# jskvrna/MonoSOWA

Measured on AMD Instinct MI355X. Metric: MonoDETR training img/s (KITTI 1280x384), higher is better.
Workload: dtype f32; 1 GPU; MonoDETR resnet50 KITTI 1280x384, fwd+criterion+bwd+AdamW step, per-GPU batch 16, synthetic images + random pseudo-labels; global_batch=16, per_gpu_batch=16, parallelism=dp1, accumulation_micro_steps=1, mixed_cameras=False, queries=550, tuned=True

## Files before the change

### include/monosowa_pointwise.h

```cpp
#ifndef MONOSOWA_POINTWISE_H_
#define MONOSOWA_POINTWISE_H_
#ifdef __cplusplus
extern "C" {
#endif

int mono_set_deterministic(int on);

int mono_bias_act_f32(float *y, const float *bias, const float *residual, long long rows, int C, int relu, void *stream);
int mono_bias_relu_maxpool_nhwc_f32(const float *y, const float *bias, float *out, int N, int H, int W, int C, void *stream);
int mono_conv1x1_tail_f32(const float *x, const float *b_in, const float *w, const float *b_out, const float *res, float *y,
                          long long M, int K, int N, void *stream);
int mono_conv1x1_tail_ds_f32(const float *x, const float *b_in, const float *w, const float *x0, const float *wd, const float *b_out,
                             float *y, long long M, int K, int N, void *stream);
int mono_conv1x1_head_f32(const float *x, const float *w, const float *b_out, float *y, long long M, int K, int N, void *stream);

int mono_relu_grad_f32(const float *grad_out, const float *y, float *grad_in, long long n, void *stream);
int mono_relu_grad_scale_f32(const float *grad_out, const float *y, const float *scale, float *grad_in, long long n, int C, void *stream);

int mono_bias_relu_mask_f32(float *y, const float *bias, const float *residual, unsigned char *mask, long long rows, int C,
                            void *stream);
int mono_relu_grad_mask_f32(const float *grad_a, const float *grad_b, const unsigned char *mask, float *grad_in, long long n,
                            void *stream);
int mono_relu_grad_mask3_f32(const float *grad_a, const float *grad_b, const float *grad_c, const unsigned char *mask, float *grad_in,
                             long long n, void *stream);

int mono_affine_relu_mask_f32(float *y, const float *scale, const float *shift, unsigned char *mask, long long rows, int C,
                              void *stream);
int mono_affine_relu_grad_f32(const float *grad, const unsigned char *mask, const float *scale, float *grad_in, long long rows,
                              int C, void *stream);

int mono_relu_grad2_f32(const float *grad_a, const float *grad_b, const float *y, float *grad_in, long long n, void *stream);
int mono_relu_grad3_f32(const float *grad_a, const float *grad_b, const float *grad_c, const float *y, float *grad_in, long long n,
                        void *stream);

int mono_dropout_add_layernorm_fwd_f32(const float *x, const float *z, const float *gamma, const float *beta, float *y,
                                       float *s, float *mean, float *rstd, long long rows, int C, float p,
                                       unsigned long long seed, float eps, void *stream);

int mono_relu_dropout_fwd_f32(const float *h, float *y, long long n, float p, unsigned long long seed, void *stream);
int mono_relu_dropout_bwd_f32(const float *grad_y, const float *y, float *grad_h, long long n, float p, void *stream);
int mono_relu_dropout_bwd_colsum_f32(const float *grad_y, const float *y, float *grad_h, float *colsum, float *partials, long long rows,
                                     float p, void *stream);

int mono_matched_losses_fwd_f32(const float *boxes, const float *depth, const float *dims, const float *angle,
                                const long long *idx, const float *t_box, const float *t_depth, const float *t_size,
                                const long long *t_bin, const float *t_res, float *out, float *comp, int NL, int B, int Q,
                                int K, void *stream);
int mono_matched_losses_bwd_f32(const float *boxes, const float *depth, const float *dims, const float *angle,
                                const long long *idx, const float *t_box, const float *t_depth, const float *t_size,
                                const long long *t_bin, const float *t_res, const float *comp, const float *grad_out,
                                float *g_boxes, float *g_depth, float *g_dims, float *g_angle, int NL, int B, int Q, int K,
                                void *stream);

int mono_adamw_step_f32(const void *table, int n_chunks, double beta1, double beta2, double eps, double step_size, void *stream);

long long mono_linear_wgrad_workspace(int R, int M, int N);
int mono_linear_wgrad_f32(const float *dy, long long ldy, const float *x, long long ldx, float *dw, float *db, float *ws, int R, int M,
                          int N, void *stream);

int mono_colsum_any_blocks(long long rows);
int mono_colsum_any_f32(const float *g, float *out, float *partials, long long rows, int C, void *stream);

// ... 69 lines not shown
```

### monosowa_amd/csrc/pointwise.hip

```cpp
#include <hip/hip_runtime.h>

#include "groupnorm.hip"
#include "matched_losses.hip"
#include "ddn_loss.hip"
#include "head_tail.hip"
#include "lsap_device.hip"
#include "conv1x1_fused.hip"
#include "small_wgrad.hip"
#include <stdint.h>
#include <algorithm>

namespace mono {

template <bool RELU, bool RES>
__global__ __launch_bounds__(256) void bias_act_kernel(float *__restrict__ y, const float *__restrict__ bias,
                                                       const float *__restrict__ residual, long long n_vec, int c_vec) {
  const long long stride = (long long)gridDim.x * blockDim.x;
  for (long long i = (long long)blockIdx.x * blockDim.x + threadIdx.x; i < n_vec; i += stride) {
    float4 v = reinterpret_cast<float4 *>(y)[i];
    const float4 b = reinterpret_cast<const float4 *>(bias)[i % c_vec];
    v.x += b.x; v.y += b.y; v.z += b.z; v.w += b.w;
    if (RES) {
      const float4 r = reinterpret_cast<const float4 *>(residual)[i];
      v.x += r.x; v.y += r.y; v.z += r.z; v.w += r.w;
    }
    if (RELU) { v.x = fmaxf(v.x, 0.f); v.y = fmaxf(v.y, 0.f); v.z = fmaxf(v.z, 0.f); v.w = fmaxf(v.w, 0.f); }
    reinterpret_cast<float4 *>(y)[i] = v;
  }
}

__global__ __launch_bounds__(256) void bias_relu_maxpool_kernel(const float *__restrict__ y, const float *__restrict__ bias,
                                                                float *__restrict__ out, int N, int H, int W, int c_vec, int OH, int OW) {
  const long long n_items = (long long)N * OH * OW * c_vec, stride = (long long)gridDim.x * blockDim.x;
  for (long long i = (long long)blockIdx.x * blockDim.x + threadIdx.x; i < n_items; i += stride) {
    const int c = (int)(i % c_vec);
    long long t = i / c_vec;
    const int ox = (int)(t % OW);
    t /= OW;
    const int oy = (int)(t % OH), n = (int)(t / OH);
    float4 m = make_float4(-INFINITY, -INFINITY, -INFINITY, -INFINITY);
#pragma unroll
    for (int dy = 0; dy < 3; ++dy) {
      const int iy = 2 * oy - 1 + dy;
      if (iy < 0 || iy >= H) continue;
#pragma unroll
      for (int dx = 0; dx < 3; ++dx) {
        const int ix = 2 * ox - 1 + dx;
        if (ix < 0 || ix >= W) continue;
        const float4 v = reinterpret_cast<const float4 *>(y)[(((long long)n * H + iy) * W + ix) * c_vec + c];
        m.x = fmaxf(m.x, v.x); m.y = fmaxf(m.y, v.y); m.z = fmaxf(m.z, v.z); m.w = fmaxf(m.w, v.w);
      }
    }
    const float4 b = reinterpret_cast<const float4 *>(bias)[c];
    reinterpret_cast<float4 *>(out)[i] = make_float4(fmaxf(m.x + b.x, 0.f), fmaxf(m.y + b.y, 0.f), fmaxf(m.z + b.z, 0.f), fmaxf(m.w + b.w, 0.f));
  }
}

template <bool RES>
__global__ __launch_bounds__(256) void bias_relu_mask_kernel(float *__restrict__ y, const float *__restrict__ bias,
                                                             const float *__restrict__ residual, unsigned char *__restrict__ mask,
// ... 455 lines not shown
      adamw_one(P.y, G.y, M.y, V.y, wd, b1, omb1, b2, omb2, eps, neg);
      adamw_one(P.z, G.z, M.z, V.z, wd, b1, omb1, b2, omb2, eps, neg);
      adamw_one(P.w, G.w, M.w, V.w, wd, b1, omb1, b2, omb2, eps, neg);
      reinterpret_cast<float4 *>(p)[i] = P; reinterpret_cast<float4 *>(m)[i] = M; reinterpret_cast<float4 *>(v)[i] = V;
    }
    for (int i = (n4 << 2) + threadIdx.x; i < n; i += 256) adamw_one(p[i], g[i], m[i], v[i], wd, b1, omb1, b2, omb2, eps, neg);
  } else {
    for (int i = threadIdx.x; i < n; i += 256) adamw_one(p[i], g[i], m[i], v[i], wd, b1, omb1, b2, omb2, eps, neg);
  }
}

inline int grid_for_vec(long long n_vec) {
  long long g = (n_vec + 255) / 256;
  if (g > 256LL * 32) g = 256LL * 32;
  return (int)(g < 1 ? 1 : g);
}

}

static int g_deterministic = 0;

extern "C" {

int mono_set_deterministic(int on) {
  const int prev = g_deterministic;
  g_deterministic = on != 0;
  return prev;
}

int mono_reduce_blocks(long long rows);

int mono_bias_act_f32(float *y, const float *bias, const float *residual, long long rows, int C, int relu, void *stream_) {
  if (!y || !bias) return -1;
  if (rows <= 0 || C <= 0 || (C & 3) || ((uintptr_t)y & 15) || ((uintptr_t)bias & 15) || ((uintptr_t)residual & 15)) return -2;
  hipStream_t stream = (hipStream_t)stream_;
  const long long n_vec = rows * C / 4;
  const int g = mono::grid_for_vec(n_vec);
  if (relu && residual) mono::bias_act_kernel<true, true><<<g, 256, 0, stream>>>(y, bias, residual, n_vec, C / 4);
  else if (relu) mono::bias_act_kernel<true, false><<<g, 256, 0, stream>>>(y, bias, nullptr, n_vec, C / 4);
  else if (residual) mono::bias_act_kernel<false, true><<<g, 256, 0, stream>>>(y, bias, residual, n_vec, C / 4);
  else mono::bias_act_kernel<false, false><<<g, 256, 0, stream>>>(y, bias, nullptr, n_vec, C / 4);
  return (int)hipGetLastError();
}

int mono_bias_relu_maxpool_nhwc_f32(const float *y, const float *bias, float *out, int N, int H, int W, int C, void *stream_) {
  if (!y || !bias || !out) return -1;
  if (N <= 0 || H <= 0 || W <= 0 || C <= 0 || (C & 3) || ((uintptr_t)y & 15) || ((uintptr_t)bias & 15) || ((uintptr_t)out & 15)) return -2;
  const int OH = (H - 1) / 2 + 1, OW = (W - 1) / 2 + 1;
  const long long n_items = (long long)N * OH * OW * (C / 4);
  mono::bias_relu_maxpool_kernel<<<mono::grid_for_vec(n_items), 256, 0, (hipStream_t)stream_>>>(y, bias, out, N, H, W, C / 4, OH, OW);
  return (int)hipGetLastError();
}

int mono_conv1x1_tail_f32(const float *x, const float *b_in, const float *w, const float *b_out, const float *res, float *y,
                          long long M, int K, int N, void *stream_) {
  if (!x || !b_in || !w || !b_out || !res || !y) return -1;
  if (M <= 0 || K != mono::kC1K || N != mono::kC1N) return -2;
  if (((uintptr_t)x & 15) || ((uintptr_t)w & 15) || ((uintptr_t)res & 15) || ((uintptr_t)y & 15)) return -2;
  if ((const float *)y == res || (const float *)y == x) return -2;
  const long long strips = (M + 31) / 32, per_wg = mono::kC1Threads / 64;
  const int grid = (int)std::min<long long>(512, (strips + per_wg - 1) / per_wg);
  mono::conv1x1_tail_kernel<<<grid, mono::kC1Threads, 0, (hipStream_t)stream_>>>(x, b_in, w, b_out, res, y, M);
  return (int)hipGetLastError();
}

int mono_conv1x1_tail_ds_f32(const float *x, const float *b_in, const float *w, const float *x0, const float *wd, const float *b_out,
                             float *y, long long M, int K, int N, void *stream_) {
  if (!x || !b_in || !w || !x0 || !wd || !b_out || !y) return -1;
  if (M <= 0 || K != mono::kC1K || N != mono::kC1N) return -2;
  if (((uintptr_t)x & 15) || ((uintptr_t)w & 15) || ((uintptr_t)x0 & 15) || ((uintptr_t)wd & 15) || ((uintptr_t)y & 15)) return -2;
  if ((const float *)y == x || (const float *)y == x0) return -2;
  const long long strips = (M + 31) / 32, per_wg = mono::kC1Threads2 / 64;
  const int grid = (int)std::min<long long>(256, (strips + per_wg - 1) / per_wg);
  mono::conv1x1_tail_ds_kernel<<<grid, mono::kC1Threads2, 0, (hipStream_t)stream_>>>(x, b_in, w, x0, wd, b_out, y, M);
  return (int)hipGetLastError();
}

int mono_conv1x1_head_f32(const float *x, const float *w, const float *b_out, float *y, long long M, int K, int N, void *stream_) {
  if (!x || !w || !b_out || !y) return -1;
  if (M <= 0 || (K != 64 && K != 256) || N != 64) return -2;
  if (((uintptr_t)x & 15) || ((uintptr_t)w & 15) || ((uintptr_t)y & 15)) return -2;
  const long long strips = (M + 31) / 32, per_wg = mono::kC1Threads / 64;
  const int grid = (int)std::min<long long>(512, (strips + per_wg - 1) / per_wg);
  if (K == 64) mono::conv1x1_head_kernel<64><<<grid, mono::kC1Threads, 0, (hipStream_t)stream_>>>(x, w, b_out, y, M);
  else mono::conv1x1_head_kernel<256><<<grid, mono::kC1Threads, 0, (hipStream_t)stream_>>>(x, w, b_out, y, M);
  return (int)hipGetLastError();
}

int mono_bias_relu_mask_f32(float *y, const float *bias, const float *residual, unsigned char *mask, long long rows, int C,
                            void *stream_) {
  if (!y || !bias || !mask) return -1;
  if (rows <= 0 || C <= 0 || (C & 3) || ((uintptr_t)y & 15) || ((uintptr_t)bias & 15) || ((uintptr_t)residual & 15)) return -2;
  const long long n_vec = rows * C / 4;
  const int g = mono::grid_for_vec(n_vec);
  if (residual) mono::bias_relu_mask_kernel<true><<<g, 256, 0, (hipStream_t)stream_>>>(y, bias, residual, mask, n_vec, C / 4);
  else mono::bias_relu_mask_kernel<false><<<g, 256, 0, (hipStream_t)stream_>>>(y, bias, nullptr, mask, n_vec, C / 4);
  return (int)hipGetLastError();
}

int mono_affine_relu_mask_f32(float *y, const float *scale, const float *shift, unsigned char *mask, long long rows, int C,
                              void *stream_) {
  if (!y || !scale || !shift || !mask) return -1;
  if (rows <= 0 || C <= 0 || (C & 3) || ((uintptr_t)y & 15) || ((uintptr_t)scale & 15) || ((uintptr_t)shift & 15)) return -2;
  const long long n_vec = rows * C / 4;
  mono::affine_relu_mask_kernel<<<mono::grid_for_vec(n_vec), 256, 0, (hipStream_t)stream_>>>(y, scale, shift, mask, n_vec, C / 4);
  return (int)hipGetLastError();
// ... 453 lines not shown
```

### monosowa_amd/monodetr/backbone.py

```python
import os

import torch
import torch.nn.functional as F
from torch import nn

from ..pointwise import (affine_relu, affine_relu_supported, bias_act, bias_act_fork, bias_relu_maxpool,
                         bias_relu_maxpool_supported, conv1x1_head, conv1x1_head_supported, conv1x1_tail,
                         conv1x1_tail_ds, conv1x1_tail_ds_supported, conv1x1_tail_supported)
from .misc import NestedTensor
from .position_encoding import build_position_encoding


AFFINE_IN_KERNEL = True
CACHE_SCALE_SHIFT = True


class FrozenBatchNorm2d(nn.Module):

    def __init__(self, n, eps=1e-5):
        super().__init__()
        self.register_buffer("weight", torch.ones(n))
        self.register_buffer("bias", torch.zeros(n))
        self.register_buffer("running_mean", torch.zeros(n))
        self.register_buffer("running_var", torch.ones(n))
        self.eps = eps

    def _load_from_state_dict(self, state_dict, prefix, local_metadata, strict, missing_keys,
                              unexpected_keys, error_msgs):
        state_dict.pop(prefix + "num_batches_tracked", None)
        super()._load_from_state_dict(state_dict, prefix, local_metadata, strict, missing_keys,
                                      unexpected_keys, error_msgs)

    def scale_shift(self):
        bufs = (self.weight, self.bias, self.running_mean, self.running_var)
        key = tuple((b.data_ptr(), b._version, b.device, b.dtype) for b in bufs)
        cached = self.__dict__.get("_scale_shift")
        if CACHE_SCALE_SHIFT and cached is not None and cached[0] == key:
            return cached[1], cached[2]
        scale = self.weight * (self.running_var + self.eps).rsqrt()
        shift = self.bias - self.running_mean * scale
        self.__dict__["_scale_shift"] = (key, scale, shift)
        return scale, shift

    def forward(self, x):
        scale, shift = self.scale_shift()
        return x * scale.reshape(1, -1, 1, 1) + shift.reshape(1, -1, 1, 1)


_PARAM_EPOCH = [0]


def _bump_param_epoch(*_args, **_kwargs):
    _PARAM_EPOCH[0] += 1


try:
    from torch.optim.optimizer import register_optimizer_step_post_hook
    register_optimizer_step_post_hook(_bump_param_epoch)
except ImportError:
    _PARAM_EPOCH = None

# ... 87 lines not shown


def conv1x1_epilogue_applies(x, conv, residual=None):
    from .. import gemm_lt
    return bool(CONV1X1_EPILOGUE & 1) and conv.kernel_size == (1, 1) and conv.stride == (1, 1) and conv.groups == 1 and conv.padding == (0, 0) \
        and x.is_cuda and x.dim() == 4 and x.dtype == torch.float32 and torch.is_grad_enabled() and conv.weight.requires_grad \
        and x.is_contiguous(memory_format=torch.channels_last) and x.shape[1] % 4 == 0 and conv.weight.shape[0] % 4 == 0 \
        and (residual is None or (residual.shape[1] == conv.weight.shape[0] and residual.is_contiguous(memory_format=torch.channels_last)
                                  and residual.dtype == torch.float32))


def conv_bn_fork(x, conv, bn, residual, n_out=2, residual_bn=None):
    if isinstance(bn, FrozenBatchNorm2d):
        scale, shift = bn.scale_shift()
        if residual_bn is not None:
            shift = _summed_shift(bn, residual_bn)
        if conv1x1_epilogue_applies(x, conv, residual):
            return _Conv1x1BnAct.apply(x, conv.weight, scale, shift, residual, n_out)
        y = conv1x1_no_grad(x, conv, scale, shift, residual, True)
        if y is not None:
            return (y,) * n_out
        y = F.conv2d(x, folded_weight(conv, bn, scale), None, conv.stride, conv.padding, conv.dilation, conv.groups)
        return bias_act_fork(y, shift, residual, n_out)
    assert residual_bn is None
    out = conv_bn(x, conv, bn, residual)
    return (out,) * n_out


def conv_bn(x, conv, bn, residual=None, relu=True):
    if isinstance(bn, FrozenBatchNorm2d):
        scale, shift = bn.scale_shift()
        if relu and residual is None and conv1x1_epilogue_applies(x, conv):
            return _Conv1x1BnAct.apply(x, conv.weight, scale, shift, None, 1)[0]
        if AFFINE_IN_KERNEL and relu and residual is None and conv.weight.requires_grad and torch.is_grad_enabled() and x.is_cuda:
            y = F.conv2d(x, conv.weight, None, conv.stride, conv.padding, conv.dilation, conv.groups)
            if affine_relu_supported(y, scale):
                return affine_relu(y, scale, shift)
            return torch.relu(y * scale.view(1, -1, 1, 1) + shift.view(1, -1, 1, 1))
        y = conv1x1_no_grad(x, conv, scale, shift, residual, relu)
        if y is not None:
            return y
        y = F.conv2d(x, folded_weight(conv, bn, scale), None, conv.stride, conv.padding, conv.dilation, conv.groups)
        return bias_act(y, shift, residual, relu)
    y = bn(conv(x))
    if residual is not None:
        y = y + residual
    return F.relu(y, inplace=True) if relu else y


FOLD_DOWNSAMPLE_SHIFT = os.environ.get("MONOSOWA_FOLD_DS_SHIFT", "1") != "0"
FUSED_FROZEN_DS = os.environ.get("MONOSOWA_FUSED_FROZEN_DS", "1") != "0"
FUSED_FROZEN_TAIL = os.environ.get("MONOSOWA_FUSED_FROZEN_TAIL", "1") != "0"
FUSED_STEM = os.environ.get("MONOSOWA_FUSED_STEM", "1") != "0"


def stem(x, conv, bn):
    if isinstance(bn, FrozenBatchNorm2d):
        scale, shift = bn.scale_shift()
        w = folded_weight(conv, bn, scale)
        if not (w.requires_grad and torch.is_grad_enabled()):
            y = F.conv2d(x, w, None, conv.stride, conv.padding, conv.dilation, conv.groups)
            if FUSED_STEM and bias_relu_maxpool_supported(y, shift):
                return bias_relu_maxpool(y, shift)
            return F.max_pool2d(bias_act(y, shift, None, True), kernel_size=3, stride=2, padding=1)
    return F.max_pool2d(conv_bn(x, conv, bn), kernel_size=3, stride=2, padding=1)


class Bottleneck(nn.Module):
    expansion = 4

    def __init__(self, inplanes, planes, stride=1, downsample=None, dilation=1, norm_layer=FrozenBatchNorm2d):
        super().__init__()
        self.conv1 = nn.Conv2d(inplanes, planes, 1, bias=False)
        self.bn1 = norm_layer(planes)
        self.conv2 = nn.Conv2d(planes, planes, 3, stride=stride, padding=dilation, dilation=dilation, bias=False)
        self.bn2 = norm_layer(planes)
        self.conv3 = nn.Conv2d(planes, planes * self.expansion, 1, bias=False)
        self.bn3 = norm_layer(planes * self.expansion)
        self.downsample = downsample

    def forward(self, x):
        xa, xb = x if isinstance(x, tuple) else (x, x)
        n_out = getattr(self, "n_out", 2)
        whole = self._frozen_block(xa, xb, n_out) if FUSED_FROZEN_TAIL else None
        if whole is not None:
            return whole
        out = conv_bn(xa, self.conv1, self.bn1)
        out = conv_bn(out, self.conv2, self.bn2)
        if self.downsample is None:
            return conv_bn_fork(out, self.conv3, self.bn3, xb, n_out)
        ds_conv, ds_bn = self.downsample[0], self.downsample[1]
        if FOLD_DOWNSAMPLE_SHIFT and isinstance(ds_bn, FrozenBatchNorm2d) and isinstance(self.bn3, FrozenBatchNorm2d):
            identity = F.conv2d(xb, folded_weight(ds_conv, ds_bn, ds_bn.scale_shift()[0]), None, ds_conv.stride, ds_conv.padding,
                                ds_conv.dilation, ds_conv.groups)
            return conv_bn_fork(out, self.conv3, self.bn3, identity, n_out, residual_bn=ds_bn)
        identity = conv_bn(xb, ds_conv, ds_bn, relu=False)
        return conv_bn_fork(out, self.conv3, self.bn3, identity, n_out)


    def _frozen_block(self, xa, xb, n_out):
        bn1, bn2, bn3, ds = self.bn1, self.bn2, self.bn3, self.downsample
        if self.conv3.weight.shape[:2] != (256, 64) or not xa.is_cuda or not isinstance(bn2, FrozenBatchNorm2d) \
                or not isinstance(bn3, FrozenBatchNorm2d) or (ds is not None and not isinstance(ds[1], FrozenBatchNorm2d)):
            return None
        if torch.is_grad_enabled() and (xa.requires_grad or xb.requires_grad or self.conv1.weight.requires_grad
                                        or self.conv2.weight.requires_grad or self.conv3.weight.requires_grad
                                        or (ds is not None and ds[0].weight.requires_grad)):
            return None
        h1 = None
        conv1 = self.conv1
        if isinstance(bn1, FrozenBatchNorm2d) and conv1.kernel_size == (1, 1) and conv1.stride == (1, 1) and conv1.weight.shape[0] == 64:
            scale1, shift1 = bn1.scale_shift()
            w1 = folded_weight(conv1, bn1, scale1)
# ... 136 lines not shown
```

### monosowa_amd/pointwise.py

```python
import ctypes
import os

import numpy as np
import torch

from . import flops
from ._lib import raw_stream, on_device, DeterministicSwitch

_PATH = os.path.join(os.path.dirname(os.path.abspath(__file__)), "lib", "libmonosowa_pointwise.so")
SYMBOLS = ("mono_bias_act_f32", "mono_bias_relu_maxpool_nhwc_f32", "mono_conv1x1_tail_f32", "mono_conv1x1_tail_ds_f32", "mono_conv1x1_head_f32", "mono_relu_grad_f32", "mono_relu_grad2_f32", "mono_relu_grad3_f32", "mono_bias_relu_mask_f32", "mono_relu_grad_mask_f32", "mono_affine_relu_mask_f32", "mono_affine_relu_grad_f32", "mono_dropout_add_layernorm_fwd_f32",
           "mono_dropout_add_layernorm_bwd_f32", "mono_groupnorm_nhwc_fwd_f32", "mono_groupnorm_nhwc_bwd_f32", "mono_groupnorm_blocks", "mono_colsum_f32", "mono_colsum_strided_f32", "mono_reduce_blocks", "mono_adamw_step_f32", "mono_relu_dropout_fwd_f32",
           "mono_relu_dropout_bwd_f32", "mono_matched_losses_fwd_f32", "mono_matched_losses_bwd_f32", "mono_ddn_loss_blocks",
           "mono_ddn_loss_fwd_f32", "mono_ddn_loss_bwd_f32", "mono_depth_expect_fwd_f32", "mono_depth_expect_bwd_f32", "mono_focal_fwd_f32", "mono_focal_bwd_f32", "mono_head_tail_fwd_f32", "mono_head_tail_bwd_f32", "mono_match_cost_f32", "mono_refine_reference_f32", "mono_relu_dropout_bwd_colsum_f32", "mono_sum_slices_f32", "mono_colsum_any_blocks", "mono_colsum_any_f32", "mono_relu_grad_mask3_f32", "mono_lsap_match_flat_f32",
           "mono_linear_wgrad_workspace", "mono_linear_wgrad_f32", "mono_colsum_levels_blocks", "mono_colsum_levels_f32", "mono_relu_grad_scale_f32",
           "mono_set_deterministic", "mono_groupnorm_stats_doubles", "mono_groupnorm_part_doubles")
_lib = None


def load():
    global _lib
    if _lib is None:
        path = os.environ.get("MONOSOWA_POINTWISE_LIB", _PATH)
        if not os.path.exists(path):
            raise RuntimeError("HIP extension %s is missing: run `python -m monosowa_amd.build`" % path)
        lib = ctypes.CDLL(path)
        P, I, LL = ctypes.c_void_p, ctypes.c_int, ctypes.c_longlong
        lib.mono_bias_act_f32.restype = I
        lib.mono_bias_act_f32.argtypes = [P, P, P, LL, I, I, P]
        lib.mono_bias_relu_maxpool_nhwc_f32.restype = I
        lib.mono_bias_relu_maxpool_nhwc_f32.argtypes = [P, P, P, I, I, I, I, P]
        lib.mono_conv1x1_tail_f32.restype = I
        lib.mono_conv1x1_tail_f32.argtypes = [P, P, P, P, P, P, LL, I, I, P]
        lib.mono_conv1x1_head_f32.restype = I
        lib.mono_conv1x1_head_f32.argtypes = [P, P, P, P, LL, I, I, P]
        lib.mono_conv1x1_tail_ds_f32.restype = I
        lib.mono_conv1x1_tail_ds_f32.argtypes = [P, P, P, P, P, P, P, LL, I, I, P]
        lib.mono_relu_grad_f32.restype = I
        lib.mono_relu_grad_f32.argtypes = [P, P, P, LL, P]
        lib.mono_relu_grad_scale_f32.restype = I
        lib.mono_relu_grad_scale_f32.argtypes = [P, P, P, P, LL, I, P]
        lib.mono_bias_relu_mask_f32.restype = I
        lib.mono_bias_relu_mask_f32.argtypes = [P, P, P, P, LL, I, P]
        lib.mono_relu_grad_mask_f32.restype = I
        lib.mono_relu_grad_mask_f32.argtypes = [P, P, P, P, LL, P]
        lib.mono_affine_relu_mask_f32.restype = I
        lib.mono_affine_relu_mask_f32.argtypes = [P, P, P, P, LL, I, P]
        lib.mono_affine_relu_grad_f32.restype = I
        lib.mono_affine_relu_grad_f32.argtypes = [P, P, P, P, LL, I, P]
        lib.mono_relu_grad2_f32.restype = I
        lib.mono_relu_grad2_f32.argtypes = [P, P, P, P, LL, P]
        lib.mono_relu_grad3_f32.restype = I
        lib.mono_relu_grad3_f32.argtypes = [P, P, P, P, P, LL, P]
        U, F = ctypes.c_ulonglong, ctypes.c_float
        lib.mono_dropout_add_layernorm_fwd_f32.restype = I
        lib.mono_dropout_add_layernorm_fwd_f32.argtypes = [P] * 8 + [LL, I, F, U, F, P]
        lib.mono_dropout_add_layernorm_bwd_f32.restype = I
        lib.mono_dropout_add_layernorm_bwd_f32.argtypes = [P] * 9 + [LL, I, F, U, P]
        lib.mono_reduce_blocks.restype = I
        lib.mono_reduce_blocks.argtypes = [LL]
        lib.mono_groupnorm_nhwc_fwd_f32.restype = I
        lib.mono_groupnorm_nhwc_fwd_f32.argtypes = [P] * 7 + [I, I, I, I, F, I, P]
        lib.mono_groupnorm_nhwc_bwd_f32.restype = I
        lib.mono_groupnorm_nhwc_bwd_f32.argtypes = [P] * 11 + [I, I, I, I, I, P]
        lib.mono_groupnorm_blocks.restype = I
        lib.mono_groupnorm_blocks.argtypes = [I, I]
        lib.mono_groupnorm_stats_doubles.restype = LL
        lib.mono_groupnorm_stats_doubles.argtypes = [I, I]
        lib.mono_groupnorm_part_doubles.restype = LL
        lib.mono_groupnorm_part_doubles.argtypes = [I, I]
        lib.mono_set_deterministic.restype = I
        lib.mono_set_deterministic.argtypes = [I]
        lib.mono_relu_dropout_fwd_f32.restype = I
        lib.mono_relu_dropout_fwd_f32.argtypes = [P, P, LL, F, U, P]
        lib.mono_colsum_any_blocks.restype = I
        lib.mono_colsum_any_blocks.argtypes = [LL]
        lib.mono_colsum_any_f32.restype = I
        lib.mono_colsum_any_f32.argtypes = [P, P, P, LL, I, P]
        lib.mono_relu_grad_mask3_f32.restype = I
        lib.mono_relu_grad_mask3_f32.argtypes = [P, P, P, P, P, LL, P]
        lib.mono_sum_slices_f32.restype = I
        lib.mono_sum_slices_f32.argtypes = [P, P, I, LL, P]
        lib.mono_relu_dropout_bwd_colsum_f32.restype = I
        lib.mono_relu_dropout_bwd_colsum_f32.argtypes = [P, P, P, P, P, LL, F, P]
# ... 172 lines not shown
                code = lib.mono_relu_grad_mask3_f32(given[0].data_ptr(), given[1].data_ptr(), given[2].data_ptr(), y.data_ptr(), g.data_ptr(), n, st)
            elif len(given) == 2:
                if ctx.masked:
                    code = lib.mono_relu_grad_mask_f32(given[0].data_ptr(), given[1].data_ptr(), y.data_ptr(), g.data_ptr(), n, st)
                else:
                    code = lib.mono_relu_grad2_f32(given[0].data_ptr(), given[1].data_ptr(), y.data_ptr(), g.data_ptr(), n, st)
            else:
                if ctx.masked:
                    code = lib.mono_relu_grad_mask_f32(given[0].data_ptr(), None, y.data_ptr(), g.data_ptr(), n, st)
                else:
                    code = lib.mono_relu_grad_f32(given[0].data_ptr(), y.data_ptr(), g.data_ptr(), n, st)
        if code:
            raise RuntimeError("mono_relu_grad(2)_f32 failed with code %d" % code)
        return g, (g.sum((0, 2, 3)) if ctx.bias_grad else None), g, None


def relu_grad_from_output(grads, y, scale=None):
    cl = lambda t: t.contiguous(memory_format=torch.channels_last)
    given = [cl(t) for t in grads]
    g = torch.empty(y.shape, dtype=torch.float32, device=y.device, memory_format=torch.channels_last)
    n = g.numel()
    lib = load()
    if scale is not None and len(given) != 1:
        raise ValueError("relu_grad_from_output: a scale goes with exactly one gradient")
    with on_device(y.device):
        if scale is not None:
            code = lib.mono_relu_grad_scale_f32(given[0].data_ptr(), y.data_ptr(), scale.data_ptr(), g.data_ptr(), n, y.shape[1], raw_stream())
        elif len(given) == 3:
            code = lib.mono_relu_grad3_f32(given[0].data_ptr(), given[1].data_ptr(), given[2].data_ptr(), y.data_ptr(), g.data_ptr(), n, raw_stream())
        elif len(given) == 2:
            code = lib.mono_relu_grad2_f32(given[0].data_ptr(), given[1].data_ptr(), y.data_ptr(), g.data_ptr(), n, raw_stream())
        else:
            code = lib.mono_relu_grad_f32(given[0].data_ptr(), y.data_ptr(), g.data_ptr(), n, raw_stream())
    if code:
        raise RuntimeError("mono_relu_grad(2)_f32 failed with code %d" % code)
    return g


def bias_relu_maxpool_supported(y, bias):
    return _nhwc_ok(y) and bias.is_cuda and bias.dtype == torch.float32 and bias.data_ptr() % 16 == 0 and bias.numel() == y.size(1) \
        and not (torch.is_grad_enabled() and (y.requires_grad or bias.requires_grad))


def bias_relu_maxpool(y, bias):
    N, C, H, W = y.shape
    out = torch.empty((N, C, (H - 1) // 2 + 1, (W - 1) // 2 + 1), dtype=torch.float32, device=y.device, memory_format=torch.channels_last)
    with on_device(y.device):
        code = load().mono_bias_relu_maxpool_nhwc_f32(y.data_ptr(), bias.data_ptr(), out.data_ptr(), N, H, W, C, raw_stream())
    if code:
        raise RuntimeError("mono_bias_relu_maxpool_nhwc_f32 failed with code %d" % code)
    return out


def conv1x1_tail_supported(x, w_kn, residual):
    return _nhwc_ok(x) and _nhwc_ok(residual) and x.size(1) == 64 and residual.size(1) == 256 and tuple(w_kn.shape) == (64, 256) \
        and x.shape[0] == residual.shape[0] and x.shape[2:] == residual.shape[2:] and w_kn.is_contiguous() and w_kn.data_ptr() % 16 == 0 \
        and not (torch.is_grad_enabled() and (x.requires_grad or residual.requires_grad or w_kn.requires_grad))


def conv1x1_tail(x, b_in, w_kn, b_out, residual):
    out = torch.empty_like(residual)
    M = x.numel() // 64
    flops.conv1x1(M, 64, 256)
    with on_device(x.device):
        code = load().mono_conv1x1_tail_f32(x.data_ptr(), b_in.data_ptr(), w_kn.data_ptr(), b_out.data_ptr(), residual.data_ptr(),
                                            out.data_ptr(), M, 64, 256, raw_stream())
    if code:
        raise RuntimeError("mono_conv1x1_tail_f32 failed with code %d" % code)
    return out


def conv1x1_tail_ds_supported(x, w_kn, x0, wd_kn):
    ok_w = lambda w: tuple(w.shape) == (64, 256) and w.is_contiguous() and w.data_ptr() % 16 == 0 and not (torch.is_grad_enabled() and w.requires_grad)
    return _nhwc_ok(x) and _nhwc_ok(x0) and x.size(1) == 64 and x0.shape == x.shape and ok_w(w_kn) and ok_w(wd_kn) \
        and not (torch.is_grad_enabled() and (x.requires_grad or x0.requires_grad))


def conv1x1_tail_ds(x, b_in, w_kn, x0, wd_kn, b_out):
    N, _, H, W = x.shape
    out = torch.empty((N, 256, H, W), dtype=torch.float32, device=x.device, memory_format=torch.channels_last)
    flops.conv1x1(N * H * W, 128, 256)
    with on_device(x.device):
        code = load().mono_conv1x1_tail_ds_f32(x.data_ptr(), b_in.data_ptr(), w_kn.data_ptr(), x0.data_ptr(), wd_kn.data_ptr(), b_out.data_ptr(),
                                               out.data_ptr(), N * H * W, 64, 256, raw_stream())
    if code:
        raise RuntimeError("mono_conv1x1_tail_ds_f32 failed with code %d" % code)
    return out


def conv1x1_head_supported(x, w_kn):
    return _nhwc_ok(x) and x.size(1) in (64, 256) and tuple(w_kn.shape) == (x.size(1), 64) and w_kn.is_contiguous() \
        and w_kn.data_ptr() % 16 == 0 and not (torch.is_grad_enabled() and (x.requires_grad or w_kn.requires_grad))


def conv1x1_head(x, w_kn, b_out):
    N, K, H, W = x.shape
    out = torch.empty((N, 64, H, W), dtype=torch.float32, device=x.device, memory_format=torch.channels_last)
    flops.conv1x1(N * H * W, K, 64)
    with on_device(x.device):
        code = load().mono_conv1x1_head_f32(x.data_ptr(), w_kn.data_ptr(), b_out.data_ptr(), out.data_ptr(), N * H * W, K, 64, raw_stream())
    if code:
        raise RuntimeError("mono_conv1x1_head_f32 failed with code %d" % code)
    return out


def bias_act_fork(y, bias, residual, n_out=2):
# ... 750 lines not shown
```

Before: 249.1 img/s.

## Fuse ResNet stem 7x7 conv, bias, ReLU and maxpool into one MFMA kernel

Adds a custom HIP kernel that computes the frozen 7x7 stride-2 stem convolution with f32 MFMA instructions, then applies the BN shift, ReLU and the 3x3 stride-2 maxpool in registers before writing the pooled NHWC output. Input rows are streamed through a shared-memory ring buffer per band/strip tile. This removes the full-resolution conv output write and re-read and the separate maxpool launch. The cost is a hand-tuned kernel with fixed tile geometry and heavy register use (two 74-entry weight arrays per lane), and it runs only when the stem is frozen.

```diff
diff --git a/include/monosowa_pointwise.h b/include/monosowa_pointwise.h
--- a/include/monosowa_pointwise.h
+++ b/include/monosowa_pointwise.h
@@ -8,6 +8,7 @@
 
 int mono_bias_act_f32(float *y, const float *bias, const float *residual, long long rows, int C, int relu, void *stream);
 int mono_bias_relu_maxpool_nhwc_f32(const float *y, const float *bias, float *out, int N, int H, int W, int C, void *stream);
+int mono_stem_conv_relu_maxpool_nhwc_f32(const float *x, const float *w, const float *shift, float *out, int N, int H, int W, void *stream);
 int mono_conv1x1_tail_f32(const float *x, const float *b_in, const float *w, const float *b_out, const float *res, float *y,
                           long long M, int K, int N, void *stream);
 int mono_conv1x1_tail_ds_f32(const float *x, const float *b_in, const float *w, const float *x0, const float *wd, const float *b_out,
diff --git a/monosowa_amd/csrc/pointwise.hip b/monosowa_amd/csrc/pointwise.hip
--- a/monosowa_amd/csrc/pointwise.hip
+++ b/monosowa_amd/csrc/pointwise.hip
@@ -6,6 +6,7 @@
 #include "head_tail.hip"
 #include "lsap_device.hip"
 #include "conv1x1_fused.hip"
+#include "stem_fused.hip"
 #include "small_wgrad.hip"
 #include <stdint.h>
 #include <algorithm>
@@ -567,6 +568,17 @@
   return (int)hipGetLastError();
 }
 
+int mono_stem_conv_relu_maxpool_nhwc_f32(const float *x, const float *w, const float *shift, float *out, int N, int H, int W, void *stream_) {
+  if (!x || !w || !shift || !out) return -1;
+  if (N <= 0 || H <= 0 || W <= 0 || ((uintptr_t)x & 3) || ((uintptr_t)w & 3) || ((uintptr_t)shift & 15) || ((uintptr_t)out & 15)) return -2;
+  const int OHc = (H - 1) / 2 + 1, OWc = (W - 1) / 2 + 1, OH = (OHc - 1) / 2 + 1, OW = (OWc - 1) / 2 + 1;
+  const int n_strips = (OW + mono::kStemStrip - 1) / mono::kStemStrip, n_bands = (OH + mono::kStemBand - 1) / mono::kStemBand;
+  const long long grid = (long long)N * n_bands * n_strips;
+  if (grid > 0x7fffffffLL) return -2;
+  mono::stem_conv_relu_maxpool_kernel<<<(int)grid, 64, 0, (hipStream_t)stream_>>>(x, w, shift, out, H, W, OHc, OWc, OH, OW, n_strips, n_bands);
+  return (int)hipGetLastError();
+}
+
 int mono_conv1x1_tail_f32(const float *x, const float *b_in, const float *w, const float *b_out, const float *res, float *y,
                           long long M, int K, int N, void *stream_) {
   if (!x || !b_in || !w || !b_out || !res || !y) return -1;
diff --git a/monosowa_amd/csrc/stem_fused.hip b/monosowa_amd/csrc/stem_fused.hip
--- /dev/null
+++ b/monosowa_amd/csrc/stem_fused.hip
@@ -0,0 +1,126 @@
+#pragma once
+#include <hip/hip_runtime.h>
+
+namespace mono {
+
+typedef float stem_f32x16 __attribute__((ext_vector_type(16)));
+constexpr int kStemRS = 208;
+constexpr int kStemBand = 6;
+constexpr int kStemStrip = 15;
+constexpr int kStemSteps = 74;
+
+__device__ constexpr int stem_k(int s, int h) { return s < 63 ? s + 21 * (s / 21) + 21 * h : (s < 73 ? 2 * s + h : 146); }
+
+__global__ __launch_bounds__(64) __attribute__((amdgpu_waves_per_eu(2, 2))) void stem_conv_relu_maxpool_kernel(const float *__restrict__ x, const float *__restrict__ w,
+                                                                    const float *__restrict__ shift, float *__restrict__ out, int H, int W,
+                                                                    int OHc, int OWc, int OH, int OW, int n_strips, int n_bands) {
+  __shared__ float ring[9 * kStemRS];
+  __shared__ float Sh[64];
+  __shared__ float4 vmax[8][64];
+  const int lane = threadIdx.x, p = lane & 31, h = lane >> 5;
+  int t = blockIdx.x;
+  const int strip = t % n_strips;
+  t /= n_strips;
+  const int band = t % n_bands, n = t / n_bands;
+  const int cb = 2 * kStemStrip * strip - 1, ix0 = 2 * cb - 3;
+  const int oy0 = band * kStemBand, oy_end = min(oy0 + kStemBand, OH);
+  const int r0 = 2 * oy0 - 1, r_end = 2 * oy_end - 1;
+  Sh[lane] = shift[lane];
+
+  float wr0[kStemSteps], wr1[kStemSteps];
+#pragma unroll
+  for (int s = 0; s < kStemSteps; ++s) {
+    const int k = h ? stem_k(s, 1) : stem_k(s, 0);
+    const bool pad = s == kStemSteps - 1 && h;
+    wr0[s] = pad ? 0.f : w[p * 147 + k];
+    wr1[s] = pad ? 0.f : w[(32 + p) * 147 + k];
+  }
+
+  bool col_ok[4];
+#pragma unroll
+  for (int m = 0; m < 4; ++m) {
+    const int i = lane + 64 * m, ix = ix0 + i / 3;
+    col_ok[m] = i < 3 * 69 && ix >= 0 && ix < W;
+  }
+  const float *xn = x + (long long)n * H * W * 3;
+  auto load_row = [&](int iy, float v[4]) {
+    const bool row_ok = iy >= 0 && iy < H;
+    const float *xr = xn + ((long long)iy * W + ix0) * 3;
+#pragma unroll
+    for (int m = 0; m < 4; ++m) v[m] = (row_ok && col_ok[m]) ? xr[lane + 64 * m] : 0.f;
+  };
+  auto store_row = [&](int iy, const float v[4]) {
+    const int slot = iy & 7;
+#pragma unroll
+    for (int m = 0; m < 4; ++m) {
+      const int i = lane + 64 * m;
+      if (i < 3 * 69) {
+        ring[slot * kStemRS + i] = v[m];
+        if (slot == 0) ring[8 * kStemRS + i] = v[m];
+      }
+    }
+  };
+  for (int ky = 0; ky < 7; ++ky) {
+    float v[4];
+    load_row(2 * r0 - 3 + ky, v);
+    store_row(2 * r0 - 3 + ky, v);
+  }
+  __syncthreads();
+
+  const int offR = 6 * p + h * kStemRS, off1 = 6 * p + h, off0 = 6 * p;
+  const bool col_valid = cb + p >= 0 && cb + p < OWc;
+  const int q = p >> 1, ox = kStemStrip * strip + q;
+  const bool writer = !(p & 1) && q < kStemStrip && ox < OW;
+  float *outp = out + 4 * h;
+#pragma unroll 1
+  for (int r = r0; r <= r_end; ++r) {
+    float nxt0[4], nxt1[4];
+    if (r < r_end) {
+      load_row(2 * r + 4, nxt0);
+      load_row(2 * r + 5, nxt1);
+    }
+    const int S0 = ((2 * r - 3) & 7) * kStemRS, S2 = ((2 * r - 1) & 7) * kStemRS, S4 = ((2 * r + 1) & 7) * kStemRS,
+              S6 = ((2 * r + 3) & 7) * kStemRS;
+    const float *b0 = ring + S0 + offR, *b2 = ring + S2 + offR, *b4 = ring + S4 + offR, *b6 = ring + S6 + off1, *b7 = ring + S6 + off0;
+    stem_f32x16 acc0 = {0.f, 0.f, 0.f, 0.f, 0.f, 0.f, 0.f, 0.f, 0.f, 0.f, 0.f, 0.f, 0.f, 0.f, 0.f, 0.f}, acc1 = acc0;
+#pragma unroll
+    for (int s = 0; s < kStemSteps; ++s) {
+      const float b = s < 21 ? b0[s] : s < 42 ? b2[s - 21] : s < 63 ? b4[s - 42] : s < 73 ? b6[2 * (s - 63)] : b7[20];
+      acc0 = __builtin_amdgcn_mfma_f32_32x32x2f32(wr0[s], b, acc0, 0, 0, 0);
+      acc1 = __builtin_amdgcn_mfma_f32_32x32x2f32(wr1[s], b, acc1, 0, 0, 0);
+    }
+    const bool valid = col_valid && r >= 0 && r < OHc;
+#pragma unroll
+    for (int j = 0; j < 8; ++j) {
+      const int nb = j >> 2, g = j & 3;
+      const float4 sh = *reinterpret_cast<const float4 *>(&Sh[32 * nb + 8 * g + 4 * h]);
+      const stem_f32x16 &acc = nb ? acc1 : acc0;
+      float4 v = make_float4(fmaxf(acc[4 * g] + sh.x, 0.f), fmaxf(acc[4 * g + 1] + sh.y, 0.f), fmaxf(acc[4 * g + 2] + sh.z, 0.f),
+                             fmaxf(acc[4 * g + 3] + sh.w, 0.f));
+      if (!valid) v = make_float4(-INFINITY, -INFINITY, -INFINITY, -INFINITY);
+      float4 &m = vmax[j][lane];
+      if (r == r0) {
+        m = v;
+      } else if (!(r & 1)) {
+        const float4 a = m;
+        m = make_float4(fmaxf(a.x, v.x), fmaxf(a.y, v.y), fmaxf(a.z, v.z), fmaxf(a.w, v.w));
+      } else {
+        const float4 a = m;
+        m = v;
+        float c[4] = {fmaxf(a.x, v.x), fmaxf(a.y, v.y), fmaxf(a.z, v.z), fmaxf(a.w, v.w)};
+#pragma unroll
+        for (int e = 0; e < 4; ++e) c[e] = fmaxf(c[e], fmaxf(__shfl_down(c[e], 1), __shfl_down(c[e], 2)));
+        if (writer)
+          *reinterpret_cast<float4 *>(outp + (((long long)n * OH + (r - 1) / 2) * OW + ox) * 64 + 32 * nb + 8 * g) = make_float4(c[0], c[1], c[2], c[3]);
+      }
+    }
+    if (r < r_end) {
+      __syncthreads();
+      store_row(2 * r + 4, nxt0);
+      store_row(2 * r + 5, nxt1);
+      __syncthreads();
+    }
+  }
+}
+
+}
diff --git a/monosowa_amd/monodetr/backbone.py b/monosowa_amd/monodetr/backbone.py
--- a/monosowa_amd/monodetr/backbone.py
+++ b/monosowa_amd/monodetr/backbone.py
@@ -6,7 +6,8 @@
 
 from ..pointwise import (affine_relu, affine_relu_supported, bias_act, bias_act_fork, bias_relu_maxpool,
                          bias_relu_maxpool_supported, conv1x1_head, conv1x1_head_supported, conv1x1_tail,
-                         conv1x1_tail_ds, conv1x1_tail_ds_supported, conv1x1_tail_supported)
+                         conv1x1_tail_ds, conv1x1_tail_ds_supported, conv1x1_tail_supported, stem_conv_relu_maxpool,
+                         stem_conv_relu_maxpool_supported)
 from .misc import NestedTensor
 from .position_encoding import build_position_encoding
 
@@ -200,6 +201,7 @@
 FUSED_FROZEN_DS = os.environ.get("MONOSOWA_FUSED_FROZEN_DS", "1") != "0"
 FUSED_FROZEN_TAIL = os.environ.get("MONOSOWA_FUSED_FROZEN_TAIL", "1") != "0"
 FUSED_STEM = os.environ.get("MONOSOWA_FUSED_STEM", "1") != "0"
+FUSED_STEM_CONV = os.environ.get("MONOSOWA_FUSED_STEM_CONV", "1") != "0"
 
 
 def stem(x, conv, bn):
@@ -207,6 +209,14 @@
         scale, shift = bn.scale_shift()
         w = folded_weight(conv, bn, scale)
         if not (w.requires_grad and torch.is_grad_enabled()):
+            if FUSED_STEM and FUSED_STEM_CONV and conv.kernel_size == (7, 7) and conv.stride == (2, 2) and conv.padding == (3, 3) \
+                    and conv.dilation == (1, 1) and conv.groups == 1 and tuple(w.shape) == (64, 3, 7, 7):
+                cached = conv.__dict__.get("_stem_w")
+                if cached is None or cached[0] is not w:
+                    with torch.no_grad():
+                        cached = conv.__dict__["_stem_w"] = (w, w.permute(0, 2, 3, 1).contiguous())
+                if stem_conv_relu_maxpool_supported(x, cached[1], shift):
+                    return stem_conv_relu_maxpool(x, cached[1], shift)
             y = F.conv2d(x, w, None, conv.stride, conv.padding, conv.dilation, conv.groups)
             if FUSED_STEM and bias_relu_maxpool_supported(y, shift):
                 return bias_relu_maxpool(y, shift)
diff --git a/monosowa_amd/pointwise.py b/monosowa_amd/pointwise.py
--- a/monosowa_amd/pointwise.py
+++ b/monosowa_amd/pointwise.py
@@ -8,7 +8,7 @@
 from ._lib import raw_stream, on_device, DeterministicSwitch
 
 _PATH = os.path.join(os.path.dirname(os.path.abspath(__file__)), "lib", "libmonosowa_pointwise.so")
-SYMBOLS = ("mono_bias_act_f32", "mono_bias_relu_maxpool_nhwc_f32", "mono_conv1x1_tail_f32", "mono_conv1x1_tail_ds_f32", "mono_conv1x1_head_f32", "mono_relu_grad_f32", "mono_relu_grad2_f32", "mono_relu_grad3_f32", "mono_bias_relu_mask_f32", "mono_relu_grad_mask_f32", "mono_affine_relu_mask_f32", "mono_affine_relu_grad_f32", "mono_dropout_add_layernorm_fwd_f32",
+SYMBOLS = ("mono_bias_act_f32", "mono_bias_relu_maxpool_nhwc_f32", "mono_stem_conv_relu_maxpool_nhwc_f32", "mono_conv1x1_tail_f32", "mono_conv1x1_tail_ds_f32", "mono_conv1x1_head_f32", "mono_relu_grad_f32", "mono_relu_grad2_f32", "mono_relu_grad3_f32", "mono_bias_relu_mask_f32", "mono_relu_grad_mask_f32", "mono_affine_relu_mask_f32", "mono_affine_relu_grad_f32", "mono_dropout_add_layernorm_fwd_f32",
            "mono_dropout_add_layernorm_bwd_f32", "mono_groupnorm_nhwc_fwd_f32", "mono_groupnorm_nhwc_bwd_f32", "mono_groupnorm_blocks", "mono_colsum_f32", "mono_colsum_strided_f32", "mono_reduce_blocks", "mono_adamw_step_f32", "mono_relu_dropout_fwd_f32",
            "mono_relu_dropout_bwd_f32", "mono_matched_losses_fwd_f32", "mono_matched_losses_bwd_f32", "mono_ddn_loss_blocks",
            "mono_ddn_loss_fwd_f32", "mono_ddn_loss_bwd_f32", "mono_depth_expect_fwd_f32", "mono_depth_expect_bwd_f32", "mono_focal_fwd_f32", "mono_focal_bwd_f32", "mono_head_tail_fwd_f32", "mono_head_tail_bwd_f32", "mono_match_cost_f32", "mono_refine_reference_f32", "mono_relu_dropout_bwd_colsum_f32", "mono_sum_slices_f32", "mono_colsum_any_blocks", "mono_colsum_any_f32", "mono_relu_grad_mask3_f32", "mono_lsap_match_flat_f32",
@@ -29,6 +29,8 @@
         lib.mono_bias_act_f32.argtypes = [P, P, P, LL, I, I, P]
         lib.mono_bias_relu_maxpool_nhwc_f32.restype = I
         lib.mono_bias_relu_maxpool_nhwc_f32.argtypes = [P, P, P, I, I, I, I, P]
+        lib.mono_stem_conv_relu_maxpool_nhwc_f32.restype = I
+        lib.mono_stem_conv_relu_maxpool_nhwc_f32.argtypes = [P, P, P, P, I, I, I, P]
         lib.mono_conv1x1_tail_f32.restype = I
         lib.mono_conv1x1_tail_f32.argtypes = [P, P, P, P, P, P, LL, I, I, P]
         lib.mono_conv1x1_head_f32.restype = I
@@ -307,6 +309,25 @@
     return out
 
 
+def stem_conv_relu_maxpool_supported(x, w_khwc, shift):
+    return x.is_cuda and x.dtype == torch.float32 and x.dim() == 4 and x.size(1) == 3 and x.is_contiguous(memory_format=torch.channels_last) \
+        and x.numel() > 0 and tuple(w_khwc.shape) == (64, 7, 7, 3) and w_khwc.dtype == torch.float32 and w_khwc.is_contiguous() \
+        and shift.is_cuda and shift.dtype == torch.float32 and shift.numel() == 64 and shift.is_contiguous() and shift.data_ptr() % 16 == 0 \
+        and not (torch.is_grad_enabled() and (x.requires_grad or w_khwc.requires_grad or shift.requires_grad))
+
+
+def stem_conv_relu_maxpool(x, w_khwc, shift):
+    N, _, H, W = x.shape
+    OH, OW = ((H - 1) // 2) // 2 + 1, ((W - 1) // 2) // 2 + 1
+    out = torch.empty((N, 64, OH, OW), dtype=torch.float32, device=x.device, memory_format=torch.channels_last)
+    with on_device(x.device):
+        code = load().mono_stem_conv_relu_maxpool_nhwc_f32(x.data_ptr(), w_khwc.data_ptr(), shift.data_ptr(), out.data_ptr(), N, H, W,
+                                                           raw_stream())
+    if code:
+        raise RuntimeError("mono_stem_conv_relu_maxpool_nhwc_f32 failed with code %d" % code)
+    return out
+
+
 def conv1x1_tail_supported(x, w_kn, residual):
     return _nhwc_ok(x) and _nhwc_ok(residual) and x.size(1) == 64 and residual.size(1) == 256 and tuple(w_kn.shape) == (64, 256) \
         and x.shape[0] == residual.shape[0] and x.shape[2:] == residual.shape[2:] and w_kn.is_contiguous() and w_kn.data_ptr() % 16 == 0 \
```

New measurement: 249.7 img/s (median of 6 runs). About the same (+0.2%).
